# joshmorgan1000/psyne

Measured on AMD Instinct MI355X. Metric: TDT encode+decode GiB/s (device-resident), 64 KiB msgs, 1/2/4/8 MI355X, higher is better.
Workload: dtype u8

## Files before the change

psyne_amd/csrc/tdt_api.hip:

```cpp
#include "../../include/psyne_tdt.h"

#include <hip/hip_runtime.h>

#include <algorithm>
#include <chrono>
#include <atomic>
#include <cstdio>
#include <cstdlib>
#include <cstring>
#include <memory>
#include <mutex>
#include <sched.h>
#include <string>
#include <vector>

#include "tdt_copypool.h"
#include "tdt_decode.h"
#include "tdt_encode.h"
#include "tdt_slots.h"

#if !defined(PSY_FAST_BUILD) && !(defined(PSY_PROF) && PSY_PROF) && !defined(PSY_SINGLE_TU)
#define PSY_ENC_EXT(WS, T, G, M, L, TL, PS, PA) \
    extern template __global__ void psy::tdt_encode_kernel<WS, T, G, psy::M, L, TL, PS, PA>(psy::EncodeArgs);
#define PSY_ENC_EXT_WS(WS)                 \
// ... 331 lines not shown
}

int ensure_elarge(PlanWS &w, int ws, hipStream_t s) {
    uint32_t lc = w.e_lcap ? w.e_lcap : kL0, tc = w.e_tcap ? w.e_tcap : kT0;
    if (w.eh.valid) {
        lc = std::max(lc, pow2_at_least(w.eh.v[4], kL0, kLmax));
        tc = std::max(tc, pow2_at_least(std::max<uint64_t>(w.eh.v[6], (uint64_t)w.eh.v[8] * psy::kSpanTiles), kT0,
                                        tile_cap_of(ws)));
    }
    if (w.elarge && lc == w.e_lcap && tc == w.e_tcap) return TDT_OK;
    if (w.elarge) {
        w.retired.push_back(w.elarge);
        w.elarge = nullptr;
        w.e_lcap = w.e_tcap = 0;
    }
    const size_t b = elarge_bytes(lc, tc, ws);
    HIPCHK(hipMalloc(&w.elarge, b));
    HIPCHK(hipMemsetAsync(w.elarge, 0, b, s));
    w.e_lcap = lc;
    w.e_tcap = tc;
    return TDT_OK;
}

template <class F>
void launch_list(uint32_t count, uint32_t team, F &&launch) {
    const uint32_t mx = 0xffffffffu / team;
    for (uint32_t b = 0; b < count; b += mx) launch(b, std::min(mx, count - b));
}

template <int WS>
int launch_slotted(tdt_ctx *c, PlanWS &pw, psy::EncodeArgs a, hipStream_t s) {
    using psy::MODE_ENCODE;
    const uint32_t n = a.n_msgs;
    int st = ensure_plan(pw, n, s);
    if (st) return st;
    const bool capturing = ::capturing(s);
    CountHist &H = pw.eh;
    if (!capturing) H.refresh();
    const bool small_on = !H.valid || H.v[10] > 0;
    const bool mid_on = !H.valid || H.v[14] > 0;
    const bool copy_on = !H.valid || H.v[18] > 0;
    bool tiles_on = !H.valid || H.v[4] > 0;
    if (tiles_on && !capturing) {
        st = ensure_elarge(pw, WS, s);
        if (st) return st;
    }
    tiles_on = tiles_on && pw.elarge;
    auto *cnt64 = reinterpret_cast<unsigned long long *>(pw.buf);
    auto *cnt = reinterpret_cast<uint32_t *>(pw.buf);
    uint32_t *slist = reinterpret_cast<uint32_t *>(pw.buf + 256), *mlist = slist + n, *qlist = mlist + n,
             *blist = qlist + n, *clist = blist + n;
    const uint32_t lcap = tiles_on ? pw.e_lcap : 0u;
    const uint32_t tcap = tiles_on ? std::min(pw.e_tcap, std::max(c->tile_cap, psy::kSpanTiles)) : 0u;
    const uint32_t scap = tcap / psy::kSpanTiles;
    auto *lmeta = reinterpret_cast<psy::LMeta *>(pw.elarge);
    auto *tiles = reinterpret_cast<uint64_t *>(pw.elarge + (size_t)pw.e_lcap * sizeof(psy::LMeta));
    auto *trec = reinterpret_cast<psy::TileRec *>(reinterpret_cast<uint8_t *>(tiles) + 8ull * pw.e_tcap);
    auto *spans =
        reinterpret_cast<uint64_t *>(reinterpret_cast<uint8_t *>(trec) + sizeof(psy::TileRec) * pw.e_tcap);
    auto *shist = reinterpret_cast<uint32_t *>(reinterpret_cast<uint8_t *>(spans) + 8ull * (pw.e_tcap / psy::kSpanTiles));
    auto *rtiles = reinterpret_cast<uint64_t *>(shist + (size_t)(pw.e_tcap / psy::kSpanTiles) * WS * 256);
    HIPCHK(hipMemsetAsync(cnt, 0, 128, s));
    psy::PlanArgs p{a.in,      a.in_off,  n,       cnt64,   slist,          mlist,              qlist,
                    blist,     clist,   tiles,   spans,          lmeta,              lcap,
                    tcap,      kSmallMax, kMidMax, kBigMin,      c->large_min,       small_on ? 1u : 0u,
                    mid_on ? 1u : 0u, a.min_tensor, (uint32_t)a.policy_on, (uint32_t)WS, copy_on ? 1u : 0u};
    const uint32_t per = psy::kPlanThreads * psy::kPlanPer;
    hipLaunchKernelGGL(psy::tdt_encode_plan_kernel, dim3((uint32_t)(((uint64_t)n + per - 1) / per)),
// ... 1616 lines not shown
```

psyne_amd/csrc/tdt_device.h:

```cpp
#pragma once
#include <hip/hip_runtime.h>
#include <stdint.h>

namespace psy {

constexpr int kWave = 64;

__device__ __forceinline__ int lane_id() { return (int)__lane_id(); }

#if defined(PSY_PROF) && PSY_PROF
__device__ unsigned long long psy_prof[32];
#define PSY_PROF_BEGIN() uint64_t psy_pt_ = __builtin_amdgcn_s_memtime()
#define PSY_PROF_MARK(i)                                                    \
    do {                                                                    \
        const uint64_t psy_t_ = __builtin_amdgcn_s_memtime();               \
        if (lane_id() == 0) atomicAdd(&psy_prof[(i)], psy_t_ - psy_pt_);    \
        psy_pt_ = psy_t_;                                                   \
    } while (0)
#elif defined(PSY_X_STOP)
#define PSY_PROF_BEGIN() ((void)0)
#define PSY_PROF_MARK(i)                        \
    do {                                        \
        if ((i) == PSY_X_STOP) return;          \
    } while (0)
#elif defined(PSY_ASM_MARKS)
#define PSY_PROF_BEGIN() ((void)0)
#define PSY_PROF_MARK(i) asm volatile(";@@MARK " #i ::)
#else
#define PSY_PROF_BEGIN() ((void)0)
#define PSY_PROF_MARK(i) ((void)0)
#endif
#ifdef PSY_ASM_MARKS
#define PSY_ASM_ROUND(p) asm volatile(";@@ROUND " #p ::)
#else
#define PSY_ASM_ROUND(p) ((void)0)
#endif

template <int CTRL, int ROWMASK = 0xf, int BANKMASK = 0xf>
__device__ __forceinline__ uint32_t dpp_mov(uint32_t x) {
    return (uint32_t)__builtin_amdgcn_update_dpp(0, (int)x, CTRL, ROWMASK, BANKMASK, false);
}

__device__ __forceinline__ int32_t med3_i32(int32_t x, int32_t lo, int32_t hi) {
    int32_t r;
    asm("v_med3_i32 %0, %1, %2, %3" : "=v"(r) : "v"(x), "v"(lo), "v"(hi));
    return r;
}

__device__ __forceinline__ uint32_t add_self(uint32_t x) {
    uint32_t r;
    asm("v_add_u32 %0, %1, %1" : "=v"(r) : "v"(x));
    return r;
}

struct OpAdd {
    __device__ __forceinline__ static uint32_t f(uint32_t a, uint32_t b) { return a + b; }
};
struct OpMax {
    __device__ __forceinline__ static uint32_t f(uint32_t a, uint32_t b) { return a > b ? a : b; }
};

template <int CTRL, int ROWMASK = 0xf, int BANKMASK = 0xf>
__device__ __forceinline__ uint32_t dpp_mov_self(uint32_t x) {
    return (uint32_t)__builtin_amdgcn_update_dpp((int)x, (int)x, CTRL, ROWMASK, BANKMASK, false);
}

template <class Op>
struct ScanIdem {
// ... 510 lines not shown
```

psyne_amd/csrc/tdt_encode.h:

```cpp
#pragma once
#include "tdt_device.h"
#include "tdt_log2.h"

#include <type_traits>

namespace psy {

static __constant__ __attribute__((aligned(16))) double c_log2_tab[128] = PSY_LOG2_TAB_INIT;
static __constant__ __attribute__((aligned(16))) double c_log2_tab2[128] = PSY_LOG2_TAB2_INIT;

enum { MODE_ENCODE = 0, MODE_MAPPED = 1, MODE_ANALYZE = 2 };

enum { ST_OK = 0, ST_SHORT = 1, ST_MAGIC = 2, ST_TRUNCATED = 3, ST_BAD_MAPPING = 4, ST_CAPACITY = 5,
       ST_UNSUPPORTED = 6, ST_BAD_HEADER = 7, ST_CONFIG = 8, ST_ARG = 11 };

constexpr uint32_t kMagicTDT = 0x54445444u;
constexpr uint32_t kMagicUNCP = 0x554E4350u;

constexpr uint32_t kNone = 0xffffffffu;
constexpr uint32_t kTileGroups = 4096;
constexpr uint32_t kSpanTiles = 8;

struct LMeta {
    uint32_t msg;
// ... 193 lines not shown
__device__ __forceinline__ uint32_t rdlane(uint32_t x, int l) {
    return (uint32_t)__builtin_amdgcn_readlane((int)x, l);
}
__device__ __forceinline__ uint32_t perm(uint32_t hi, uint32_t lo, uint32_t sel) {
    return __builtin_amdgcn_perm(hi, lo, sel);
}
__host__ __device__ constexpr uint32_t sb_pos(uint32_t j) { return 8u * (j >> 2) + (j & 3u); }
__host__ __device__ constexpr uint32_t sb_slot(uint32_t b) { return ((b >> 3) << 2) | (b & 3u); }
__device__ __forceinline__ uint32_t sb_spread(uint32_t x) {
    return (x & 0xfu) | ((x & 0xf0u) << 4) | ((x & 0xf00u) << 8) | ((x & 0xf000u) << 12);
}
__device__ __forceinline__ uint32_t sb_compact(uint32_t x) {
    x = (x | (x >> 4)) & 0x00ff00ffu;
    return (x | (x >> 8)) & 0xffffu;
}
__device__ __forceinline__ uint32_t spread2(uint32_t e) {
    uint32_t x = e & 0xffffu;
    x = (x | (x << 8)) & 0x00ff00ffu;
    x = (x | (x << 4)) & 0x0f0f0f0fu;
    x = (x | (x << 2)) & 0x33333333u;
    x = (x | (x << 1)) & 0x55555555u;
    return x | (x << 1);
}

#ifndef PSY_ENC_WPE
#define PSY_ENC_WPE 8
#endif
#ifndef PSY_ENC_LDAUX
#define PSY_ENC_LDAUX 0
#endif
#ifndef PSY_ENC_WPE_LB
#define PSY_ENC_WPE_LB 6
#endif
#define PSY_ENC_WAVES(TEAM, LB) ((TEAM) >= 512 ? ((LB) ? PSY_ENC_WPE_LB : PSY_ENC_WPE) : (TEAM) >= 256 ? 6 : 7)

enum { PATH_BOTH = 0, PATH_RES = 1, PATH_STREAM = 2 };

template <int WS, int TEAM, int G, int MODE, int LB, int TL, int PATH = PATH_BOTH>
__device__ __forceinline__ void encode_one(const EncodeArgs &a, uint8_t *smem, uint32_t msg, uint32_t lj,
                                           uint32_t tile) {
    static_assert(TL == 0 || (TEAM * G == (int)kTileGroups && MODE == MODE_ENCODE && !LB), "tile shape");
    constexpr uint32_t kTG = TL == 1 ? kTileGroups * kSpanTiles : kTileGroups;
    using Lay = EncLayout<WS, TEAM, LB>;
    constexpr int W = Lay::W;
    constexpr int WPG = Lay::WPG;
    uint32_t *slots = reinterpret_cast<uint32_t *>(smem + Lay::OFF_SLOTS);
    uint32_t *misc = reinterpret_cast<uint32_t *>(smem + Lay::OFF_MISC);
    const int tid = threadIdx.x;
    const int lane = lane_id();
    const int wv = __builtin_amdgcn_readfirstlane(tid >> 6);
    PSY_PROF_BEGIN();

    if (msg >= a.n_msgs) return;
    PSY_PROF_MARK(0);

    const uint64_t off0 = a.in_off[msg];
    const uint64_t n = a.in_off[msg + 1] - off0;
    const uint8_t *base = a.in + off0;
    uint64_t slot_b = 0, slot_e = 0;
    if constexpr (!LB) {
        slot_b = a.slot_off[msg];
        slot_e = a.slot_off[msg + 1];
    }

    auto place = [&](uint64_t E, bool &fits) __attribute__((always_inline)) -> uint64_t {
        uint64_t ob;
        if constexpr (LB) {
            if (wv == 0) {
#ifndef PSY_X_NOLB
                const uint64_t b = lookback_excl_wave(a.lookback, msg, E, a.errflags);
#else
// ... 63 lines not shown
        const LMeta &lm = a.lmeta[lj];
        if (lm.mapbits == kSpec && a.trec[lm.tile0 + tile].clean != kRecount) return;
    }

    const uint32_t n32 = (uint32_t)n;
    const uint32_t wc = n32 / WS;
    const uint32_t ngroups = (n32 + 15) / 16;
    const uint32_t tg0 = TL ? tile * kTG : 0u;
    const uint32_t tgn = TL == 4 ? 0u : TL ? umin(ngroups - tg0, kTG) : ngroups;
    const uint32_t RW = TL == 1 && SPECA1 ? kTileGroups / 64u : (tgn + TEAM - 1) / TEAM;
    const bool al16 = ((uintptr_t)base & 15) == 0;
    const bool resident = TL != 4 && RW <= (uint32_t)G && al16 && (n32 & 15u) == 0;
    const uint32_t gw0 = tg0 + (uint32_t)wv * RW * 64;

    auto vbytes = [&](uint32_t g) __attribute__((always_inline)) -> uint32_t {
        const int64_t vb64 = (int64_t)n32 - 16 * (int64_t)g;
        return vb64 >= 16 ? 16u : (vb64 <= 0 ? 0u : (uint32_t)vb64);
    };
    auto load_group = [&](uint32_t g) __attribute__((always_inline)) -> uint4 {
        const uint32_t vb = vbytes(g);
        if (vb == 16 && al16) return *reinterpret_cast<const uint4 *>(base + 16ull * g);
        if (vb == 0) return make_uint4(0, 0, 0, 0);
        return ld16_any(base + 16ull * g, (int)vb);
    };
    const uint32_t nfull = n32 >> 4;
    auto full_round = [&](uint32_t r) __attribute__((always_inline)) -> bool {
        return gw0 + r * 64u + 64u <= nfull;
    };

    auto run = [&](auto res_tag) __attribute__((always_inline)) {
    constexpr bool RES = decltype(res_tag)::value;
    constexpr int GR = RES ? G : 1;
    uint4 dres[GR];
    uint32_t cres[GR];
    constexpr int NL2 = W == 1 ? 1 : (128 + TEAM - 1) / TEAM;
    uint4 l2v[NL2];
    if constexpr (MODE != MODE_MAPPED && W > 1) {
#pragma unroll
        for (int k = 0; k < NL2; ++k) {
            const int i = (tid + k * TEAM) & 127;
            l2v[k] = reinterpret_cast<const uint4 *>(i < 64 ? c_log2_tab : c_log2_tab2)[i & 63];
        }
    }
    if constexpr (RES) {
        const __amdgpu_buffer_rsrc_t rsrc =
            __builtin_amdgcn_make_buffer_rsrc(const_cast<uint8_t *>(base), (short)0, (int)n32, 0x00020000);
        const int vo = (int)((gw0 + (uint32_t)lane) * 16u);
#pragma unroll
        for (int r = 0; r < G; ++r) {
            typedef unsigned int u32x4_t __attribute__((ext_vector_type(4)));
            const u32x4_t v = __builtin_amdgcn_raw_buffer_load_b128(rsrc, vo, r * 1024, PSY_ENC_LDAUX);
            dres[r] = make_uint4(v.x, v.y, v.z, v.w);
            cres[r] = 0;
        }
    }
    auto for_rounds = [&](auto &&body) __attribute__((always_inline)) {
        if constexpr (RES) {
#pragma unroll
            for (int r = 0; r < G; ++r)
                if ((uint32_t)r < RW) body((uint32_t)r, dres[r], cres[r], std::true_type{});
        } else {
            auto live = [&](uint32_t r) __attribute__((always_inline)) {
                return r < RW && gw0 + r * 64u < ngroups;
            };
            if constexpr (PF == 1) {
                for (uint32_t r = 0; live(r); ++r) {
                    uint4 d = load_group(gw0 + r * 64 + lane);
                    uint32_t c = 0;
                    body(r, d, c, std::false_type{});
                }
            } else {
                uint4 q[PF];
#pragma unroll
                for (int k = 0; k < PF; ++k) q[k] = live((uint32_t)k) ? load_group(gw0 + k * 64 + lane) : uint4{};
                bool go = true;
                for (uint32_t r0 = 0; go; r0 += PF) {
#pragma unroll
                    for (int k = 0; k < PF; ++k) {
                        const uint32_t r = r0 + (uint32_t)k;
                        if (!live(r)) {
                            go = false;
                            break;
                        }
                        uint4 d = q[k];
                        if (live(r + PF)) q[k] = load_group(gw0 + (r + PF) * 64 + lane);
                        uint32_t c = 0;
                        body(r, d, c, std::false_type{});
                    }
                }
            }
        }
    };

// ... 409 lines not shown
            const uint64_t mb = (uint64_t)msg * WS;
            if (tid < WS) {
                if (a.ent_out) a.ent_out[mb + tid] = reinterpret_cast<const double *>(wm + M_ENT)[tid];
                if (a.map_out) a.map_out[mb + tid] = (int32_t)wm[M_MAP + tid];
            }
            if (tid == 0 && a.status) a.status[msg] = ST_OK;
            return;
        }
        if constexpr (TL == 4) {
            uint32_t bits = 0;
            for (int b = 0; b < WS; ++b) bits |= wm[M_MAP + b] << b;
            if (tid == 0) a.lmeta[lj].mapbits = bits;
            {
                const uint32_t nt = a.lmeta[lj].ntiles, t0 = a.lmeta[lj].tile0;
                const bool miss = kSpec == 0xffffffffu || bits != kSpec;
                for (uint32_t t = (uint32_t)tid; t < nt; t += TEAM) {
                    const bool need = miss || a.trec[t0 + t].clean == kRecount;
                    const uint64_t bal = __ballot(need);
                    if (bal == 0) continue;
                    const int first = __ffsll((unsigned long long)bal) - 1;
                    uint32_t base = 0;
                    if (lane == first) base = (uint32_t)atomicAdd(a.rcount, (unsigned long long)__popcll(bal));
                    base = (uint32_t)__shfl((int)base, first);
                    const uint32_t rank = __builtin_amdgcn_mbcnt_hi((uint32_t)(bal >> 32),
                                                                    __builtin_amdgcn_mbcnt_lo((uint32_t)bal, 0u));
                    if (need) a.rtiles[base + rank] = ((uint64_t)t << 32) | lj;
                }
            }
            return;
        }
    }

    if constexpr (MODE != MODE_ANALYZE) {
        uint32_t ns, L0, k0, k1, selA[4], selB[4], edA, edB;
        const uint32_t mapbits = __builtin_amdgcn_readfirstlane(wm[M_MAPBITS]);
        if constexpr (WS <= 8) {
            const SlotLayout &SL = slot_layout<WS>(mapbits);
            ns = SL.ns;
            L0 = SL.L0;
            k0 = SL.k0;
            k1 = SL.k1;
#pragma unroll
            for (int q = 0; q < 4; ++q) {
                selA[q] = SL.selA[q];
                selB[q] = SL.selB[q];
            }
            edA = SL.edA;
            edB = SL.edB;
        } else {
            if (tid < 16) {
                uint32_t k[2] = {0, 0};
                for (int b = 0; b < WS; ++b) k[wm[M_MAP + b]]++;
                const uint32_t L0w = WPG * k[0];
                const uint32_t j = (uint32_t)lane;
                const uint32_t c = j < L0w ? 0u : 1u;
                const uint32_t jj = c ? j - L0w : j;
                const uint32_t rank = jj % k[c];
                uint32_t b = 0, seen = 0;
                for (int bb = 0; bb < WS; ++bb) {
                    if (wm[M_MAP + bb] == c) {
                        if (seen == rank) b = bb;
                        ++seen;
                    }
                }
                wm[M_SB + j] = (jj / k[c]) * WS + b;
                if (j == 0) {
                    wm[M_NS] = k[1] ? 2u : 1u;
                    wm[M_L0] = L0w;
                    wm[M_K0] = k[0];
// ... 4 lines not shown
            if (tid < 5) {
                const uint32_t L0w = wm[M_L0];
                const bool two = wm[M_NS] == 2;
                uint32_t A = 0x0c0c0c0cu, B = 0x0c0c0c0cu;
                for (int t = 0; t < 4; ++t) {
                    uint32_t sv = 0xffu;
                    if (lane < 4) sv = wm[M_SB + 4 * t + lane];
                    else if (t == 0 && L0w > 0) sv = wm[M_SB + L0w - 1];
                    else if (t == 1) sv = wm[M_SB + 15];
                    else if (t == 2 && two) sv = wm[M_SB + L0w];
                    if (sv == 0xffu) continue;
                    if (sv < 8) A = (A & ~(0xffu << (8 * t))) | (sv << (8 * t));
                    else B = (B & ~(0xffu << (8 * t))) | ((sv - 8) << (8 * t));
                }
                wm[lane < 4 ? M_SELA + lane : M_EDA] = A;
                wm[lane < 4 ? M_SELB + lane : M_EDB] = B;
            }
            team_sync<W>();
            ns = __builtin_amdgcn_readfirstlane(wm[M_NS]);
            L0 = __builtin_amdgcn_readfirstlane(wm[M_L0]);
            k0 = __builtin_amdgcn_readfirstlane(wm[M_K0]);
            k1 = __builtin_amdgcn_readfirstlane(wm[M_K1]);
#pragma unroll
            for (int q = 0; q < 4; ++q) {
                selA[q] = __builtin_amdgcn_readfirstlane(wm[M_SELA + q]);
                selB[q] = __builtin_amdgcn_readfirstlane(wm[M_SELB + q]);
            }
            edA = __builtin_amdgcn_readfirstlane(wm[M_EDA]);
            edB = __builtin_amdgcn_readfirstlane(wm[M_EDB]);
        }
        const bool ns2 = ns == 2;
        const uint32_t Ls[2] = {L0, ns2 ? 16u - L0 : 0u};
        const uint32_t lowL0 = L0 >= 16 ? 0xffffu : ((1u << L0) - 1u);
        constexpr bool BL = RES && WS <= 4 && TL != 2;
        const uint32_t lowX = BL ? sb_spread(lowL0) : lowL0;
        const uint32_t highX = BL ? sb_spread(~lowL0 & 0xffffu) : (~lowL0 & 0xffffu);
        const uint32_t fullX = BL ? 0x0f0f0f0fu : 0xffffu;
        uint32_t fsA = 0x0c0c0c0cu, fsB = 0x0c0c0c0cu;
        if (ns2) {
            const uint32_t q = L0 & 3u, t = L0 >> 2, sel = 0x0c0c0c00u | ((q & 1u) * 4u + t);
            if (q < 2) fsA = sel;
            else fsB = sel;
        }
        PSY_PROF_MARK(2);

        auto tmat = [&](const uint4 &d, uint32_t (&T)[4]) __attribute__((always_inline)) {
#pragma unroll
            for (int q = 0; q < 4; ++q) T[q] = perm(d.y, d.x, selA[q]) | perm(d.w, d.z, selB[q]);
        };
        auto edges = [&](const uint4 &d) __attribute__((always_inline)) -> uint32_t {
            return perm(d.y, d.x, edA) | perm(d.w, d.z, edB);
        };
        auto vmask = [&](uint32_t vb) __attribute__((always_inline)) -> uint32_t {
            const uint32_t nvw = vb / WS;
            if (nvw >= (uint32_t)WPG) return 0xffffu;
            uint32_t v = (1u << (nvw * k0)) - 1u;
            if (ns2) v |= ((1u << (nvw * k1)) - 1u) << L0;
            return v;
        };
        constexpr bool kFold = WS <= 4;
        const uint32_t p0sel = kFold && ns2 ? (0x06050400u & ~(0xffu << (2u * L0))) | (0x01u << (2u * L0)) : 0x06050400u;
        auto run_mask = [&](const uint32_t (&T)[4], uint32_t ed, uint32_t edc, bool first, uint32_t V,
                            auto blm) __attribute__((always_inline)) -> uint32_t {
            constexpr bool BLM = decltype(blm)::value;
            const uint32_t pe = wave_shr1(ed, edc);
            const uint32_t P0 = perm(T[3], pe, p0sel);
            const uint32_t X[4] = {T[0] ^ P0, T[1] ^ T[0], T[2] ^ T[1], T[3] ^ T[2]};
// ... 67 lines not shown
        };

        uint32_t edc0 = 0;
        if (gw0 > 0 && gw0 - 1 < ngroups) edc0 = __builtin_amdgcn_readfirstlane(edges(load_group(gw0 - 1)));

        uint32_t wmax[2] = {0, 0};
        uint32_t lr[2] = {0, 0};
        uint64_t lb[2] = {0ull, 0ull};
        uint64_t zk1[2], zk8[2];
#pragma unroll
        for (int c = 0; c < 2; ++c) {
            const bool b8 = Ls[c] < 16u;
            zk1[c] = b8 ? 0x0101010101010101ull : 0x1111111111111111ull;
            zk8[c] = Ls[c] == 0u ? 0ull : b8 ? 0x8080808080808080ull : 0x8888888888888888ull;
        }
        uint64_t zacc = 0;
        uint32_t pc0 = 0, pc1 = 0;
        uint32_t fmx[2] = {0, 0};
        const uint32_t gL[2] = {(gw0 + (uint32_t)lane) * Ls[0], (gw0 + (uint32_t)lane) * Ls[1]};
        bool spec_hit = false;
        if constexpr (SPEC_ON && TL == 0) {
            spec_hit = mapbits == kSpec;
            if (spec_hit) {
                wmax[0] = s_wmax[0];
                wmax[1] = s_wmax[1];
                pc0 = s_pc0;
                pc1 = s_pc1;
                zacc = s_zacc;
            }
        }
        if (!spec_hit) {
            uint32_t edc = edc0;
            for_rounds([&](uint32_t r, uint4 &d, uint32_t &cm, auto res) __attribute__((always_inline)) {
                PSY_ASM_ROUND(A1);
                const uint32_t g = gw0 + r * 64 + lane;
                const uint32_t ed = edges(d);
                uint32_t T[4];
                tmat(d, T);
                const uint32_t V = full_round(r) ? fullX : (BL ? sb_spread(vmask(vbytes(g))) : vmask(vbytes(g)));
                const uint32_t m = run_mask(T, ed, edc, r == 0u && gw0 == 0u, V, std::integral_constant<bool, BL>{});
                edc = rdlane(ed, 63);
                cm = m;
                if constexpr (decltype(res)::value) d = make_uint4(T[0], T[1], T[2], T[3]);
                constexpr bool SW = decltype(res)::value && TL != 2;
                const uint32_t m0 = m & lowX;
                const uint64_t r0 = (uint64_t)__ballot(m0 != 0u);
                if constexpr (SW) {
                    if (r0) {
                        lr[0] = r;
                        lb[0] = r0;
                    }
                } else {
                    if (m0) wmax[0] = umax(wmax[0], gL[0] + r * 64u * Ls[0] + hibit(m0) + 1u);
                }
                pc0 += popc(m0);
                if constexpr (TL == 2) {
                    if (m0) fmx[0] = umax(fmx[0], ~(g * Ls[0] + lobit(m0)));
                }
                const uint64_t pastm = full_round(r) ? 0ull : (uint64_t)__ballot(g >= ngroups);
                const uint64_t b0 = r0 | pastm;
                zacc |= (b0 - zk1[0]) & ~b0 & zk8[0];
                if (ns2) {
                    const uint32_t m1 = BL ? m & highX : m >> L0;
                    const uint64_t r1 = (uint64_t)__ballot(m > lowX);
                    if constexpr (SW) {
                        if (r1) {
                            lr[1] = r;
                            lb[1] = r1;
                        }
                    } else {
                        if (m1) wmax[1] = umax(wmax[1], gL[1] + r * 64u * Ls[1] + hibit(m1) + 1u);
                    }
                    pc1 += popc(m1);
                    if constexpr (TL == 2) {
                        if (m1) fmx[1] = umax(fmx[1], ~(g * Ls[1] + lobit(m1)));
                    }
                    const uint64_t b1 = r1 | pastm;
                    zacc |= (b1 - zk1[1]) & ~b1 & zk8[1];
                }
            });
        }
        if constexpr (RES && TL != 2) {
#pragma unroll
            for (int c = 0; c < 2; ++c) {
                if (lb[c] == 0ull) continue;
                const uint32_t l = 63u - (uint32_t)__builtin_clzll(lb[c]);
                uint32_t mv = 0;
#pragma unroll
                for (int r = 0; r < GR; ++r)
                    if ((uint32_t)r == lr[c]) mv = rdlane(cres[r], (int)l);
                uint32_t hb;
                if constexpr (BL) hb = sb_slot(hibit(c ? mv & highX : mv & lowX)) - (c ? L0 : 0u);
                else hb = hibit(c ? mv >> L0 : mv & lowL0);
                wmax[c] = (gw0 + lr[c] * 64u + l) * Ls[c] + hb + 1u;
            }
        } else {
            wmax[0] = wave_reduce<OpMax>(wmax[0]);
            wmax[1] = wave_reduce<OpMax>(wmax[1]);
        }
        if constexpr (TL == 2) {
            fmx[0] = wave_reduce<OpMax>(fmx[0]);
            fmx[1] = wave_reduce<OpMax>(fmx[1]);
        }
        pc0 = wave_reduce<OpAdd>(pc0);
        pc1 = ns2 ? wave_reduce<OpAdd>(pc1) : 0u;
        if (lane == 0) {
            slots[wv * 8 + 0] = wmax[0];
            slots[wv * 8 + 1] = wmax[1];
            slots[wv * 8 + 2] = pc0;
            slots[wv * 8 + 3] = pc1;
            slots[wv * 8 + 5] = zacc != 0ull ? 1u : 0u;
            if constexpr (TL == 2) {
                slots[wv * 8 + 6] = fmx[0];
                slots[wv * 8 + 7] = fmx[1];
            }
        }
        team_sync<W>();
        uint32_t rin[2] = {0, 0};
        uint32_t capped = 0;
        const TileRec *tr = nullptr;
        if constexpr (TL == 3) {
            tr = a.trec + a.lmeta[lj].tile0 + tile;
            rin[0] = tr->lrs[0];
            rin[1] = tr->lrs[1];
            capped = tr->clean ? 0u : 1u;
        }
#pragma unroll
        for (int ww = 0; ww < W; ++ww) {
            if (ww < wv) {
                rin[0] = umax(rin[0], slots[ww * 8 + 0]);
                rin[1] = umax(rin[1], slots[ww * 8 + 1]);
            }
            capped |= slots[ww * 8 + 5];
        }
        rin[0] = __builtin_amdgcn_readfirstlane(rin[0]);
        rin[1] = __builtin_amdgcn_readfirstlane(rin[1]);
        const bool clean = __builtin_amdgcn_readfirstlane(capped) == 0u;
        PSY_PROF_MARK(3);

        if (!clean) {
            pc0 = pc1 = 0;
            uint32_t rcarry[2] = {rin[0], rin[1]};
            uint32_t edc = edc0;
            for_rounds([&](uint32_t r, uint4 &d, uint32_t &cm, auto res) __attribute__((always_inline)) {
                PSY_ASM_ROUND(A2);
                const uint32_t g = gw0 + r * 64 + lane;
                const uint32_t V = full_round(r) ? 0xffffu : vmask(vbytes(g));
                uint32_t m;
                if constexpr (decltype(res)::value) {
                    m = BL ? sb_compact(cm) : cm;
                } else {
                    uint32_t T[4];
                    tmat(d, T);
                    const uint32_t ed = edges(d);
                    m = run_mask(T, ed, edc, r == 0u && gw0 == 0u, V, std::false_type{});
                    edc = rdlane(ed, 63);
                }
                const uint32_t C = chunk_round(r, m, rcarry, g, V);
                cm = BL ? sb_spread(C) : C;
                pc0 += popc(C & lowL0);
                pc1 += popc(C >> L0);
            });
            pc0 = wave_reduce<OpAdd>(pc0);
            pc1 = ns2 ? wave_reduce<OpAdd>(pc1) : 0u;
            if (lane == 0) {
                slots[wv * 8 + 2] = pc0;
                slots[wv * 8 + 3] = pc1;
            }
            team_sync<W>();
        }
        PSY_PROF_MARK(4);
        uint32_t pin[2] = {0, 0}, ptot[2] = {0, 0};
#pragma unroll
        for (int ww = 0; ww < W; ++ww) {
            const uint32_t s0 = slots[ww * 8 + 2], s1 = slots[ww * 8 + 3];
            if (ww < wv) {
                pin[0] += s0;
                pin[1] += s1;
            }
            ptot[0] += s0;
            ptot[1] += s1;
        }
        if constexpr (TL == 2) {
            if (tid == 0) {
                uint32_t l[2] = {0, 0}, f[2] = {0, 0};
                for (int ww = 0; ww < W; ++ww) {
                    l[0] = umax(l[0], slots[ww * 8 + 0]);
                    l[1] = umax(l[1], slots[ww * 8 + 1]);
                    f[0] = umax(f[0], slots[ww * 8 + 6]);
                    f[1] = umax(f[1], slots[ww * 8 + 7]);
                }
                TileRec *t = a.trec + a.lmeta[lj].tile0 + tile;
// ... 61 lines not shown
        uint32_t ccarry[2] = {0, 0};
#pragma unroll
        for (int c = 0; c < 2; ++c) {
            const uint32_t W0 = gw0 * Ls[c];
            if (rin[c] && W0 > 0) {
                const uint32_t rs = rin[c] - 1;
                ccarry[c] = rs + 255u * ((W0 - 1 - rs) / 255u) + 1u;
            }
        }


        uint32_t pi5[2] = {0, 0}, pend[2] = {0, 0};
        bool hp[2] = {false, false};
#pragma unroll
        for (int c = 0; c < 2; ++c) {
            if (c == 1 && !ns2) break;
            const uint32_t p_in = __builtin_amdgcn_readfirstlane(pin[c]);
            if (p_in > 0 && ccarry[c] > 0) {
                hp[c] = true;
                pi5[c] = p_in - 1;
                const uint32_t val = (edc0 >> (8 * c)) & 0xffu;
                pend[c] = (val << 24) | (ccarry[c] - 1u + 256u - gw0 * Ls[c]);
            }
        }
        const uint32_t slen[2] = {wc * k0, wc * k1};
        const uint32_t ebase = wst + 256u;
        const uint32_t jl = wst;
        const uint32_t eoff1 = 4u * (1u + 64u * L0);
        const uint32_t pb0 = (uint32_t)lane * Ls[0] + 256u, pb1 = (uint32_t)lane * Ls[1] + 256u - L0;
        auto emit5 = [&](uint32_t r, const uint4 &Tw, uint32_t C) __attribute__((always_inline)) {
#ifdef PSY_X_NOEMIT
            if (r < 100) return;
#endif
            PSY_ASM_ROUND(B);
            const uint32_t T[4] = {Tw.x, Tw.y, Tw.z, Tw.w};
            const uint32_t gr = gw0 + r * 64;
            const uint32_t c0 = popc(C & lowL0);
            const uint32_t pc = c0 | (popc(C >> L0) << 16);
            const uint32_t pinc = wave_incl_scan<OpAdd>(pc);
            const uint32_t pexc = pinc - pc;
            const uint32_t Stot = rdlane(pinc, 63);
            const uint32_t S[2] = {Stot & 0xffffu, Stot >> 16};
            if (lane == 0) {
                if (hp[0]) *reinterpret_cast<uint32_t *>(smem + ebase) = pend[0];
                if (ns2 && hp[1]) *reinterpret_cast<uint32_t *>(smem + ebase + eoff1) = pend[1];
            }
            const uint32_t D0 = ebase + 4u * (1u + (pexc & 0xffffu)) - jl;
            const uint32_t D1 = ebase + eoff1 + 4u * (1u + (pexc >> 16)) - jl;
            uint32_t D = L0 == 0 ? D1 : D0;
#pragma unroll
            for (int j = 0; j < 16; ++j) {
                const int q = j & 3, t = j >> 2;
                if (j > 0 && j % WPG == 0 && (uint32_t)j == L0) D = D1;
                const bool s0 = (uint32_t)j < L0;
                const uint32_t bit = (C >> j) & 1u;
                const uint32_t pos = (s0 ? pb0 : pb1) + (uint32_t)j;
                uint32_t ad;
                asm("v_mad_u32_u24 %0, %1, %2, %3" : "=v"(ad) : "v"(bit), "v"(D), "v"(jl));
                *reinterpret_cast<uint32_t *>(smem + ad) =
                    perm(T[q], pos, ((uint32_t)(4 + t) << 24) | 0x000c0100u);
                asm("v_lshl_add_u32 %0, %1, 2, %2" : "=v"(D) : "v"(bit), "v"(D));
            }
            team_sync<1>();
            const bool last = gr <= ngroups - 1 && ngroups - 1 < gr + 64;
#pragma unroll
            for (int c = 0; c < 2; ++c) {
                if (c == 1 && !ns2) break;
// ... 52 lines not shown
            }
            team_sync<1>();
        };

        constexpr bool E6 = RES && WS <= 4;
        constexpr bool E6S = WS <= 4;
        const uint32_t eb6 = wst + 16u;
        constexpr uint32_t NB = Lay::NB6;
        const uint32_t eoff6 = 2u * (2u + NB * 64u * L0);
        uint32_t u6[2] = {hp[0] ? 1u : 0u, hp[1] ? 1u : 0u};
        uint32_t pend6[2] = {0, 0};
#pragma unroll
        for (int c = 0; c < 2; ++c) pend6[c] = ((pend[c] >> 24) << 8) | ((pend[c] - 256u + gw0 * Ls[c]) & 0xffu);
        uint32_t pos6[4] = {0, 0, 0, 0};
        if constexpr (E6S) {
            const uint32_t A4 = perm(0u, pb0, 0x00000000u), B4 = perm(0u, pb1, 0x00000000u);
#pragma unroll
            for (int q = 0; q < 4; ++q) {
                uint32_t mq = 0;
#pragma unroll
                for (int t = 0; t < 4; ++t) mq |= (4u * t + q < L0 ? 0xffu : 0u) << (8 * t);
                const uint32_t x = (A4 & mq) | (B4 & ~mq);
                const uint32_t jq = 0x0c080400u + (uint32_t)q * 0x01010101u;
                pos6[q] = ((x & 0x7f7f7f7fu) + jq) ^ (x & 0x80808080u);
            }
        }
        auto scan6 = [&](uint32_t C, uint32_t &pexc, uint32_t &Stot) __attribute__((always_inline)) {
            const uint32_t pc = popc(C & lowX) | (popc(C & highX) << 16);
            const uint32_t pinc = wave_incl_scan<OpAdd>(pc);
            pexc = pinc - pc;
            Stot = __builtin_amdgcn_readfirstlane(rdlane(pinc, 63));
        };
        auto sweep6 = [&](const uint4 &Tw, uint32_t C, uint32_t pexc, uint32_t Stot) __attribute__((always_inline)) {
            PSY_ASM_ROUND(B);
            const uint32_t T[4] = {Tw.x, Tw.y, Tw.z, Tw.w};
            const uint32_t D0 = eb6 + 2u * (u6[0] + (pexc & 0xffffu)) - jl;
            const uint32_t D1 = eb6 + eoff6 + 2u * (u6[1] + (pexc >> 16)) - jl;
            uint32_t D = L0 == 0 ? D1 : D0;
            uint32_t E[4][2];
#pragma unroll
            for (int q = 0; q < 4; ++q) {
                E[q][0] = perm(T[q], pos6[q], 0x05010400u);
                E[q][1] = perm(T[q], pos6[q], 0x07030602u);
            }
#pragma unroll
            for (int j = 0; j < 16; ++j) {
                const int q = j & 3, t = j >> 2;
                if (j > 0 && j % WPG == 0 && (uint32_t)j == L0) D = D1;
                const uint32_t bit = (C >> (BL ? sb_pos(j) : j)) & 1u;
                uint32_t ad;
                asm("v_mad_u32_u24 %0, %1, %2, %3" : "=v"(ad) : "v"(bit), "v"(D), "s"(jl));
                const uint32_t e = E[q][t >> 1];
                if (t & 1) *reinterpret_cast<uint16_t *>(smem + ad) = (uint16_t)(e >> 16);
                else *reinterpret_cast<uint16_t *>(smem + ad) = (uint16_t)e;
                asm("v_lshl_add_u32 %0, %1, 1, %2" : "=v"(D) : "v"(bit), "v"(D));
            }
            u6[0] += Stot & 0xffffu;
            u6[1] += Stot >> 16;
        };
        auto flush6 = [&](bool last) __attribute__((always_inline)) {
#if defined(PSY_X_NOEMIT) || defined(PSY_X_NOFLUSH)
            if (ngroups != 0xffffffffu) { u6[0] = u6[1] = 0; return; }
#endif
            team_sync<1>();
#pragma unroll
            for (int c = 0; c < 2; ++c) {
                if (c == 1 && !ns2) break;
                const uint32_t nent = u6[c];
                const uint32_t K = nent ? nent - 1u : 0u;
                const uint32_t eb = eb6 + (c ? eoff6 : 0u);
                uint8_t *const Dp = dst + sdata[c] + 2ull * pi5[c];
                auto pair_at = [&](uint32_t k) __attribute__((always_inline)) -> uint32_t {
                    const uint32_t e0 = *reinterpret_cast<const uint16_t *>(smem + eb + 2u * k);
                    const uint32_t e1 = *reinterpret_cast<const uint16_t *>(smem + eb + 2u * k + 2u);
                    return perm(e0, e1 - e0, 0x0c0c0500u);
                };
// ... 96 lines not shown
                        misc[M_BASE + 2] = ok;
                        __builtin_amdgcn_fence(__ATOMIC_RELEASE, "workgroup");
                        __hip_atomic_store(&wm[M_READY], 1u, __ATOMIC_RELAXED, __HIP_MEMORY_SCOPE_WORKGROUP);
                    }
                } else {
                    while (__hip_atomic_load(&wm[M_READY], __ATOMIC_RELAXED, __HIP_MEMORY_SCOPE_WORKGROUP) == 0u)
                        __builtin_amdgcn_s_sleep(2);
                    __builtin_amdgcn_fence(__ATOMIC_ACQUIRE, "workgroup");
                    b = *reinterpret_cast<const uint64_t *>(misc + M_BASE);
                    ok = misc[M_BASE + 2];
                }
                b = rfl_u64(b);
                dst = a.out + b;
                return __builtin_amdgcn_readfirstlane(ok) != 0u;
            };
            uint32_t rb = 0;
            auto flush_batch = [&](uint32_t re) __attribute__((always_inline)) -> bool {
                if constexpr (DEFER) {
                    if (!resolved) {
                        resolved = true;
                        if (!resolve_lb()) return false;
                    }
                }
                const uint32_t gb = gw0 + rb * 64u, ge = gw0 + re * 64u;
                flush6(gb <= ngroups - 1 && ngroups - 1 < ge);
                fresh = true;
                rb = re;
                return true;
            };
#pragma unroll
            for (int r = 0; r < G; ++r) {
                if ((uint32_t)r < RW) {
                    uint32_t pexc, Stot;
                    scan6(cres[r], pexc, Stot);
                    const uint32_t over = (u6[0] + (Stot & 0xffffu) > cap6[0] ? 1u : 0u) |
                                          (u6[1] + (Stot >> 16) > cap6[1] ? 1u : 0u);
                    if (over != 0u && !fresh) {
                        if (!flush_batch((uint32_t)r)) return;
                    }
                    if (fresh && lane == 0) {
                        if (u6[0]) *reinterpret_cast<uint16_t *>(smem + eb6) = (uint16_t)pend6[0];
                        if (ns2 && u6[1]) *reinterpret_cast<uint16_t *>(smem + eb6 + eoff6) = (uint16_t)pend6[1];
                    }
                    fresh = false;
#ifndef PSY_X_NOEMIT
                    sweep6(dres[r], cres[r], pexc, Stot);
#endif
                    if ((uint32_t)(r + 1) == RW) {
                        if (!flush_batch((uint32_t)r + 1u)) return;
                    }
                }
            }
          } else
          {
#pragma unroll
            for (int r = 0; r < G; ++r) {
                if ((uint32_t)r < RW) {
                    emit5((uint32_t)r, dres[r], cres[r]);
                }
            }
          }
        } else {
            uint32_t rcarry[2] = {rin[0], rin[1]};
            uint32_t edc = edc0;
            auto chunk_of = [&](uint32_t r, const uint4 &d, uint4 &Tw) __attribute__((always_inline)) -> uint32_t {
                const uint32_t g = gw0 + r * 64 + lane;
                const uint32_t V = full_round(r) ? 0xffffu : vmask(vbytes(g));
                uint32_t T[4];
                tmat(d, T);
                Tw = make_uint4(T[0], T[1], T[2], T[3]);
                const uint32_t ed = edges(d);
                const uint32_t m = run_mask(T, ed, edc, r == 0u && gw0 == 0u, V, std::false_type{});
                edc = rdlane(ed, 63);
                return clean ? m : chunk_round(r, m, rcarry, g, V);
            };
            uint4 Tc;
            uint32_t Cc = chunk_of(0, load_group(gw0 + lane), Tc);
            if constexpr (E6S) {
                const uint32_t cap6[2] = {1u + NB * 64u * Ls[0], 1u + NB * 64u * Ls[1]};
                bool fresh = true;
                uint32_t rb = 0;
                for (uint32_t r = 0; r < RW; ++r) {
                    uint4 Tn = make_uint4(0, 0, 0, 0);
                    uint32_t Cn = 0;
                    if (r + 1 < RW) Cn = chunk_of(r + 1, load_group(gw0 + (r + 1) * 64 + lane), Tn);
                    uint32_t pexc, Stot;
                    scan6(Cc, pexc, Stot);
                    const uint32_t over = (u6[0] + (Stot & 0xffffu) > cap6[0] ? 1u : 0u) |
                                          (u6[1] + (Stot >> 16) > cap6[1] ? 1u : 0u);
                    if (over != 0u && !fresh) {
                        const uint32_t gb = gw0 + rb * 64u, ge = gw0 + r * 64u;
                        flush6(gb <= ngroups - 1 && ngroups - 1 < ge);
                        fresh = true;
                        rb = r;
                    }
                    if (fresh && lane == 0) {
                        if (u6[0]) *reinterpret_cast<uint16_t *>(smem + eb6) = (uint16_t)pend6[0];
                        if (ns2 && u6[1]) *reinterpret_cast<uint16_t *>(smem + eb6 + eoff6) = (uint16_t)pend6[1];
                    }
                    fresh = false;
                    sweep6(Tc, Cc, pexc, Stot);
                    if (r + 1 == RW) {
                        const uint32_t gb = gw0 + rb * 64u, ge = gw0 + r * 64u + 64u;
                        flush6(gb <= ngroups - 1 && ngroups - 1 < ge);
                        fresh = true;
                        rb = r + 1u;
                    }
                    Tc = Tn;
                    Cc = Cn;
                }
            } else {
                for (uint32_t r = 0; r < RW; ++r) {
                    uint4 Tn = make_uint4(0, 0, 0, 0);
                    uint32_t Cn = 0;
                    if (r + 1 < RW) Cn = chunk_of(r + 1, load_group(gw0 + (r + 1) * 64 + lane), Tn);
                    emit5(r, Tc, Cc);
                    Tc = Tn;
                    Cc = Cn;
                }
            }
        }
        PSY_PROF_MARK(6);
    }
    };
    if constexpr (PATH == PATH_RES) {
        if (resident) {
            run(std::true_type{});
        } else if (tid == 0) {
            atomicOr(a.errflags, 8u);
            if (a.status) a.status[msg] = ST_ARG;
            if (a.out_len) a.out_len[msg] = 0;
        }
    } else if constexpr (PATH == PATH_STREAM) {
        run(std::false_type{});
    } else {
        if (resident) run(std::true_type{});
        else run(std::false_type{});
    }
}

template <int TL>
__device__ __forceinline__ uint32_t entry_count(const EncodeArgs &a) {
    uint32_t c;
    if constexpr (TL == 0) c = *a.list_count + (a.list2 ? *a.list2_count : 0u);
    else if constexpr (TL == 4) c = umin(a.pcnt[4], a.lcap);
    else if constexpr (TL == 1) c = umin(a.pcnt[8], a.tcap / kSpanTiles);
    else if constexpr (TL == 2) c = umin(a.pcnt[22], a.tcap);
    else c = umin(a.pcnt[6], a.tcap);
    return __builtin_amdgcn_readfirstlane(c);
}

template <int WS, int TEAM, int G, int MODE, int LB, int TL = 0, int PS = 0, int PATH = PATH_BOTH>
__global__ __launch_bounds__(TEAM, PSY_ENC_WAVES(TEAM, LB)) void tdt_encode_kernel(EncodeArgs a) {
    using Lay = EncLayout<WS, TEAM, LB>;
    constexpr int W = Lay::W;
    __shared__ __attribute__((aligned(16))) uint8_t smem[Lay::BYTES];
    if constexpr (LB) {
        uint32_t *misc = reinterpret_cast<uint32_t *>(smem + Lay::OFF_MISC);
        if (threadIdx.x == 0) misc[M_MSG] = atomicAdd(a.ticket, 1u);
        team_sync<W>();
        encode_one<WS, TEAM, G, MODE, LB, 0>(a, smem, __builtin_amdgcn_readfirstlane(misc[M_MSG]), 0, 0);
        return;
    } else {
        const uint32_t n2 = TL == 0 && a.list2 ? __builtin_amdgcn_readfirstlane(*a.list2_count) : 0u;
        auto one = [&](uint32_t i) __attribute__((always_inline)) {
            if constexpr (TL == 0) {
                encode_one<WS, TEAM, G, MODE, LB, 0, PATH>(a, smem, i < n2 ? a.list2[i] : a.list[i - n2], 0, 0);
            } else if constexpr (TL == 4) {
                const uint32_t msg = a.lmeta[i].msg;
                if (msg != kNone) encode_one<WS, TEAM, G, MODE, LB, TL>(a, smem, msg, i, 0);
            } else {
                const uint64_t e = TL == 1 ? a.spans[i] : TL == 2 ? a.rtiles[i] : a.tiles[i];
                const uint32_t lj = (uint32_t)e;
                if (lj == kNone) return;
                encode_one<WS, TEAM, G, MODE, LB, TL>(a, smem, a.lmeta[lj].msg, lj, (uint32_t)(e >> 32));
            }
        };
        const uint32_t cnt = entry_count<TL>(a);
        const uint32_t i0 = a.list_base + blockIdx.x;
        if constexpr (PS) {
            for (uint32_t i = i0; i < cnt; i += gridDim.x) {
                if (i != i0) team_sync<W>();
                one(i);
            }
        } else if constexpr (TL == 0) {
            const uint32_t ic = i0 < a.n_msgs ? i0 : a.n_msgs - 1u;
            const uint32_t e2 = a.list2 ? a.list2[ic] : 0u, e1 = a.list[ic];
            if (i0 >= cnt) return;
            encode_one<WS, TEAM, G, MODE, LB, 0, PATH>(a, smem, i0 < n2 ? e2 : (n2 == 0u ? e1 : a.list[i0 - n2]), 0,
                                                       0);
        } else {
            if (i0 >= cnt) return;
            one(i0);
        }
    }
}

struct PlanArgs {
    const uint8_t *in;
    const uint64_t *in_off;
    uint32_t n_msgs;
    unsigned long long *cnt;
    uint32_t *slist, *mlist, *qlist, *blist, *clist;
    uint64_t *tiles, *spans;
    LMeta *lmeta;
    uint32_t lmax, tile_cap;
    uint64_t small_max, mid_max, big_min, large_min;
    uint32_t small_on;
    uint32_t mid_on;
    uint64_t min_tensor;
    uint32_t policy_on, ws;
    uint32_t copy_on;
};

constexpr uint32_t kPlanThreads = 1024, kPlanPer = 2;

#ifndef PSY_ENC_INST_TU
__global__ __launch_bounds__(kPlanThreads) void tdt_encode_plan_kernel(PlanArgs p) {
    __shared__ uint64_t lds[8 * (kPlanPer * 16 + 1)];
    const uint32_t scap = p.tile_cap / kSpanTiles;
    uint64_t thr = p.large_min;
    if (p.n_msgs) {
        const uint64_t share = (p.in_off[p.n_msgs] - p.in_off[0]) / 4096;
// ... 171 lines not shown
```

Measured before the change: 1165.

## Specialize encode post-phase on expected mapbits and pack per-round masks

Adds a dual-path post phase for WS=4, TEAM=512 resident encode. When the runtime map bits equal a compile-time expected value (kSpec), it uses a constexpr slot layout, otherwise it falls back to the generic path. The per-round chunk masks are packed two per register using nibble-spread layouts, and pos6 offsets are derived with immediate adds, both to cut VGPR pressure. The final flush now happens once after all rounds, and argument checks are added on the host. Risks are larger code from duplicated instantiations and extra shift/mask work per round.

```diff
diff --git a/psyne_amd/csrc/tdt_api.hip b/psyne_amd/csrc/tdt_api.hip
--- a/psyne_amd/csrc/tdt_api.hip
+++ b/psyne_amd/csrc/tdt_api.hip
@@ -387,8 +387,10 @@
 int launch_slotted(tdt_ctx *c, PlanWS &pw, psy::EncodeArgs a, hipStream_t s) {
     using psy::MODE_ENCODE;
     const uint32_t n = a.n_msgs;
+    if (n == 0) return set_err(TDT_E_ARG, "slotted encode launch without messages");
     int st = ensure_plan(pw, n, s);
     if (st) return st;
+    if (pw.bytes < 256 + 20ull * n) return set_err(TDT_E_ARG, "plan buffer smaller than five lists of n entries");
     const bool capturing = ::capturing(s);
     CountHist &H = pw.eh;
     if (!capturing) H.refresh();
diff --git a/psyne_amd/csrc/tdt_device.h b/psyne_amd/csrc/tdt_device.h
--- a/psyne_amd/csrc/tdt_device.h
+++ b/psyne_amd/csrc/tdt_device.h
@@ -32,8 +32,14 @@
 #endif
 #ifdef PSY_ASM_MARKS
 #define PSY_ASM_ROUND(p) asm volatile(";@@ROUND " #p ::)
+#define PSY_ASM_ROUND_L(cl, p)             \
+    do {                                   \
+        if constexpr (cl) PSY_ASM_ROUND(p##c); \
+        else PSY_ASM_ROUND(p);             \
+    } while (0)
 #else
 #define PSY_ASM_ROUND(p) ((void)0)
+#define PSY_ASM_ROUND_L(cl, p) ((void)0)
 #endif
 
 template <int CTRL, int ROWMASK = 0xf, int BANKMASK = 0xf>
diff --git a/psyne_amd/csrc/tdt_encode.h b/psyne_amd/csrc/tdt_encode.h
--- a/psyne_amd/csrc/tdt_encode.h
+++ b/psyne_amd/csrc/tdt_encode.h
@@ -249,11 +249,14 @@
 #ifndef PSY_ENC_WPE_LB
 #define PSY_ENC_WPE_LB 6
 #endif
+#ifndef PSY_ENC_DUAL
+#define PSY_ENC_DUAL 1
+#endif
 #define PSY_ENC_WAVES(TEAM, LB) ((TEAM) >= 512 ? ((LB) ? PSY_ENC_WPE_LB : PSY_ENC_WPE) : (TEAM) >= 256 ? 6 : 7)
 
 enum { PATH_BOTH = 0, PATH_RES = 1, PATH_STREAM = 2 };
 
-template <int WS, int TEAM, int G, int MODE, int LB, int TL, int PATH = PATH_BOTH>
+template <int WS, int TEAM, int G, int MODE, int LB, int TL, int PATH = PATH_BOTH, bool CARM = false>
 __device__ __forceinline__ void encode_one(const EncodeArgs &a, uint8_t *smem, uint32_t msg, uint32_t lj,
                                            uint32_t tile) {
     static_assert(TL == 0 || (TEAM * G == (int)kTileGroups && MODE == MODE_ENCODE && !LB), "tile shape");
@@ -383,7 +386,16 @@
     constexpr bool RES = decltype(res_tag)::value;
     constexpr int GR = RES ? G : 1;
     uint4 dres[GR];
-    uint32_t cres[GR];
+    constexpr bool kBLR = RES && WS <= 4 && TL != 2;
+    constexpr uint32_t kCS = kBLR ? 4u : 16u, kCM = kBLR ? 0x0f0f0f0fu : 0xffffu;
+    uint32_t cres[(GR + 1) / 2];
+    auto cget = [&](uint32_t cm, uint32_t r) __attribute__((always_inline)) -> uint32_t {
+        return RES ? (cm >> (kCS * (r & 1u))) & kCM : cm;
+    };
+    auto cput = [&](uint32_t &cm, uint32_t r, uint32_t m) __attribute__((always_inline)) {
+        if constexpr (RES) cm = (cm & ~(kCM << (kCS * (r & 1u)))) | (m << (kCS * (r & 1u)));
+        else cm = m;
+    };
     constexpr int NL2 = W == 1 ? 1 : (128 + TEAM - 1) / TEAM;
     uint4 l2v[NL2];
     if constexpr (MODE != MODE_MAPPED && W > 1) {
@@ -393,6 +405,7 @@
             l2v[k] = reinterpret_cast<const uint4 *>(i < 64 ? c_log2_tab : c_log2_tab2)[i & 63];
         }
     }
+    auto load_rounds = [&]() __attribute__((always_inline)) {
     if constexpr (RES) {
         const __amdgpu_buffer_rsrc_t rsrc =
             __builtin_amdgcn_make_buffer_rsrc(const_cast<uint8_t *>(base), (short)0, (int)n32, 0x00020000);
@@ -402,14 +415,16 @@
             typedef unsigned int u32x4_t __attribute__((ext_vector_type(4)));
             const u32x4_t v = __builtin_amdgcn_raw_buffer_load_b128(rsrc, vo, r * 1024, PSY_ENC_LDAUX);
             dres[r] = make_uint4(v.x, v.y, v.z, v.w);
-            cres[r] = 0;
+            cres[r >> 1] = 0;
         }
     }
+    };
+    load_rounds();
     auto for_rounds = [&](auto &&body) __attribute__((always_inline)) {
         if constexpr (RES) {
 #pragma unroll
             for (int r = 0; r < G; ++r)
-                if ((uint32_t)r < RW) body((uint32_t)r, dres[r], cres[r], std::true_type{});
+                if ((uint32_t)r < RW) body((uint32_t)r, dres[r], cres[r >> 1], std::true_type{});
         } else {
             auto live = [&](uint32_t r) __attribute__((always_inline)) {
                 return r < RW && gw0 + r * 64u < ngroups;
@@ -885,9 +900,29 @@
     }
 
     if constexpr (MODE != MODE_ANALYZE) {
+        constexpr bool DUAL = CARM && RES && kSpec != 0xffffffffu;
+        auto post = [&](auto ltag) __attribute__((always_inline)) {
+        constexpr bool CL = decltype(ltag)::value;
+        int lane_ = lane_id();
+        if constexpr (RES) asm volatile("v_mbcnt_lo_u32_b32 %0, -1, 0\n\tv_mbcnt_hi_u32_b32 %0, -1, %0" : "=v"(lane_));
+        const int lane = lane_;
+        const int tid = RES ? wv * 64 + lane_ : (int)threadIdx.x;
         uint32_t ns, L0, k0, k1, selA[4], selB[4], edA, edB;
-        const uint32_t mapbits = __builtin_amdgcn_readfirstlane(wm[M_MAPBITS]);
-        if constexpr (WS <= 8) {
+        const uint32_t mapbits = CL ? kSpec : __builtin_amdgcn_readfirstlane(wm[M_MAPBITS]);
+        if constexpr (CL) {
+            constexpr SlotLayout CS = make_slot_layout<WS>(kSpec);
+            ns = CS.ns;
+            L0 = CS.L0;
+            k0 = CS.k0;
+            k1 = CS.k1;
+#pragma unroll
+            for (int q = 0; q < 4; ++q) {
+                selA[q] = CS.selA[q];
+                selB[q] = CS.selB[q];
+            }
+            edA = CS.edA;
+            edB = CS.edB;
+        } else if constexpr (WS <= 8) {
             const SlotLayout &SL = slot_layout<WS>(mapbits);
             ns = SL.ns;
             L0 = SL.L0;
@@ -958,7 +993,7 @@
         const bool ns2 = ns == 2;
         const uint32_t Ls[2] = {L0, ns2 ? 16u - L0 : 0u};
         const uint32_t lowL0 = L0 >= 16 ? 0xffffu : ((1u << L0) - 1u);
-        constexpr bool BL = RES && WS <= 4 && TL != 2;
+        constexpr bool BL = kBLR;
         const uint32_t lowX = BL ? sb_spread(lowL0) : lowL0;
         const uint32_t highX = BL ? sb_spread(~lowL0 & 0xffffu) : (~lowL0 & 0xffffu);
         const uint32_t fullX = BL ? 0x0f0f0f0fu : 0xffffu;
@@ -1092,7 +1127,7 @@
         if (!spec_hit) {
             uint32_t edc = edc0;
             for_rounds([&](uint32_t r, uint4 &d, uint32_t &cm, auto res) __attribute__((always_inline)) {
-                PSY_ASM_ROUND(A1);
+                PSY_ASM_ROUND_L(CL, A1);
                 const uint32_t g = gw0 + r * 64 + lane;
                 const uint32_t ed = edges(d);
                 uint32_t T[4];
@@ -1100,7 +1135,7 @@
                 const uint32_t V = full_round(r) ? fullX : (BL ? sb_spread(vmask(vbytes(g))) : vmask(vbytes(g)));
                 const uint32_t m = run_mask(T, ed, edc, r == 0u && gw0 == 0u, V, std::integral_constant<bool, BL>{});
                 edc = rdlane(ed, 63);
-                cm = m;
+                cput(cm, r, m);
                 if constexpr (decltype(res)::value) d = make_uint4(T[0], T[1], T[2], T[3]);
                 constexpr bool SW = decltype(res)::value && TL != 2;
                 const uint32_t m0 = m & lowX;
@@ -1148,7 +1183,7 @@
                 uint32_t mv = 0;
 #pragma unroll
                 for (int r = 0; r < GR; ++r)
-                    if ((uint32_t)r == lr[c]) mv = rdlane(cres[r], (int)l);
+                    if ((uint32_t)r == lr[c]) mv = rdlane(cget(cres[r >> 1], (uint32_t)r), (int)l);
                 uint32_t hb;
                 if constexpr (BL) hb = sb_slot(hibit(c ? mv & highX : mv & lowX)) - (c ? L0 : 0u);
                 else hb = hibit(c ? mv >> L0 : mv & lowL0);
@@ -1203,12 +1238,12 @@
             uint32_t rcarry[2] = {rin[0], rin[1]};
             uint32_t edc = edc0;
             for_rounds([&](uint32_t r, uint4 &d, uint32_t &cm, auto res) __attribute__((always_inline)) {
-                PSY_ASM_ROUND(A2);
+                PSY_ASM_ROUND_L(CL, A2);
                 const uint32_t g = gw0 + r * 64 + lane;
                 const uint32_t V = full_round(r) ? 0xffffu : vmask(vbytes(g));
                 uint32_t m;
                 if constexpr (decltype(res)::value) {
-                    m = BL ? sb_compact(cm) : cm;
+                    m = BL ? sb_compact(cget(cm, r)) : cget(cm, r);
                 } else {
                     uint32_t T[4];
                     tmat(d, T);
@@ -1217,7 +1252,7 @@
                     edc = rdlane(ed, 63);
                 }
                 const uint32_t C = chunk_round(r, m, rcarry, g, V);
-                cm = BL ? sb_spread(C) : C;
+                cput(cm, r, BL ? sb_spread(C) : C);
                 pc0 += popc(C & lowL0);
                 pc1 += popc(C >> L0);
             });
@@ -1345,7 +1380,7 @@
 #ifdef PSY_X_NOEMIT
             if (r < 100) return;
 #endif
-            PSY_ASM_ROUND(B);
+            PSY_ASM_ROUND_L(CL, B);
             const uint32_t T[4] = {Tw.x, Tw.y, Tw.z, Tw.w};
             const uint32_t gr = gw0 + r * 64;
             const uint32_t c0 = popc(C & lowL0);
@@ -1464,16 +1499,22 @@
             Stot = __builtin_amdgcn_readfirstlane(rdlane(pinc, 63));
         };
         auto sweep6 = [&](const uint4 &Tw, uint32_t C, uint32_t pexc, uint32_t Stot) __attribute__((always_inline)) {
-            PSY_ASM_ROUND(B);
+            PSY_ASM_ROUND_L(CL, B);
             const uint32_t T[4] = {Tw.x, Tw.y, Tw.z, Tw.w};
             const uint32_t D0 = eb6 + 2u * (u6[0] + (pexc & 0xffffu)) - jl;
             const uint32_t D1 = eb6 + eoff6 + 2u * (u6[1] + (pexc >> 16)) - jl;
             uint32_t D = L0 == 0 ? D1 : D0;
             uint32_t E[4][2];
+            uint32_t pq[4] = {pos6[0], pos6[1], pos6[2], pos6[3]};
+            if constexpr (RES) {
+                asm volatile("v_add_u32_e32 %0, 0x01010101, %1" : "=v"(pq[1]) : "v"(pos6[0]));
+                asm volatile("v_add_u32_e32 %0, 0x02020202, %1" : "=v"(pq[2]) : "v"(pos6[0]));
+                asm volatile("v_add_u32_e32 %0, 0x03030303, %1" : "=v"(pq[3]) : "v"(pos6[0]));
+            }
 #pragma unroll
             for (int q = 0; q < 4; ++q) {
-                E[q][0] = perm(T[q], pos6[q], 0x05010400u);
-                E[q][1] = perm(T[q], pos6[q], 0x07030602u);
+                E[q][0] = perm(T[q], pq[q], 0x05010400u);
+                E[q][1] = perm(T[q], pq[q], 0x07030602u);
             }
 #pragma unroll
             for (int j = 0; j < 16; ++j) {
@@ -1636,7 +1677,8 @@
             for (int r = 0; r < G; ++r) {
                 if ((uint32_t)r < RW) {
                     uint32_t pexc, Stot;
-                    scan6(cres[r], pexc, Stot);
+                    const uint32_t Cr = cget(cres[r >> 1], (uint32_t)r);
+                    scan6(Cr, pexc, Stot);
                     const uint32_t over = (u6[0] + (Stot & 0xffffu) > cap6[0] ? 1u : 0u) |
                                           (u6[1] + (Stot >> 16) > cap6[1] ? 1u : 0u);
                     if (over != 0u && !fresh) {
@@ -1648,19 +1690,17 @@
                     }
                     fresh = false;
 #ifndef PSY_X_NOEMIT
-                    sweep6(dres[r], cres[r], pexc, Stot);
+                    sweep6(dres[r], Cr, pexc, Stot);
 #endif
-                    if ((uint32_t)(r + 1) == RW) {
-                        if (!flush_batch((uint32_t)r + 1u)) return;
-                    }
-                }
-            }
+                }
+            }
+            if (!flush_batch(RW)) return;
           } else
           {
 #pragma unroll
             for (int r = 0; r < G; ++r) {
                 if ((uint32_t)r < RW) {
-                    emit5((uint32_t)r, dres[r], cres[r]);
+                    emit5((uint32_t)r, dres[r], cget(cres[r >> 1], (uint32_t)r));
                 }
             }
           }
@@ -1725,6 +1765,14 @@
             }
         }
         PSY_PROF_MARK(6);
+        };
+        if constexpr (DUAL) {
+            if (__builtin_expect_with_probability(__builtin_amdgcn_readfirstlane(wm[M_MAPBITS]) == kSpec, 1, 0.999))
+                post(std::true_type{});
+            else post(std::false_type{});
+        } else {
+            post(std::false_type{});
+        }
     }
     };
     if constexpr (PATH == PATH_RES) {
@@ -1791,8 +1839,9 @@
             const uint32_t ic = i0 < a.n_msgs ? i0 : a.n_msgs - 1u;
             const uint32_t e2 = a.list2 ? a.list2[ic] : 0u, e1 = a.list[ic];
             if (i0 >= cnt) return;
-            encode_one<WS, TEAM, G, MODE, LB, 0, PATH>(a, smem, i0 < n2 ? e2 : (n2 == 0u ? e1 : a.list[i0 - n2]), 0,
-                                                       0);
+            constexpr bool CARM = PSY_ENC_DUAL && WS == 4 && TEAM == 512 && PATH == PATH_RES && MODE == MODE_ENCODE;
+            encode_one<WS, TEAM, G, MODE, LB, 0, PATH, CARM>(a, smem, i0 < n2 ? e2 : (n2 == 0u ? e1 : a.list[i0 - n2]),
+                                                             0, 0);
         } else {
             if (i0 >= cnt) return;
             one(i0);
```

Result: faster. 1199, median of 6 (+2.9%).
